# yangjunjie0320/fft-isdf-scratch

Measured on AMD Instinct MI355X. Metric: ISDF build + get_jk k-points/s, diamond gth-dzvp 4x4x4, higher is better.
Workload: dtype f64 (complex128)

## Files before the change

fft-isdf-scratch_amd/csrc/fft.hip:

```cpp
#include <type_traits>

#include "common.h"

typedef double fft_dv2 __attribute__((ext_vector_type(2)));


#include <map>
#include <mutex>
#include <vector>
#include <cmath>

namespace fisdf {

namespace {

constexpr int MAXN = 64;
constexpr int MAXST = 8;

struct Stages {
  int nst;
  int radix[MAXST];
};

template <int R>
__device__ __forceinline__ void dft_small(cplx* v, const cplx* __restrict__ tw, int n) {
  if constexpr (R == 2) {
    cplx a = v[0], b = v[1];
    v[0] = cadd(a, b);
    v[1] = csub(a, b);
  } else if constexpr (R == 4) {
    cplx a0 = cadd(v[0], v[2]), a1 = csub(v[0], v[2]);
    cplx b0 = cadd(v[1], v[3]), b1 = csub(v[1], v[3]);
    cplx b1m = cmk(b1.y, -b1.x);
    v[0] = cadd(a0, b0);
    v[2] = csub(a0, b0);
    v[1] = cadd(a1, b1m);
    v[3] = csub(a1, b1m);
  } else {
    cplx o[R];
    const int step = n / R;
#pragma unroll
    for (int k = 0; k < R; ++k) {
      cplx acc = v[0];
#pragma unroll
      for (int r = 1; r < R; ++r) acc = cadd(acc, cmul(v[r], tw[((r * k) % R) * step]));
      o[k] = acc;
    }
#pragma unroll
    for (int k = 0; k < R; ++k) v[k] = o[k];
  }
}

template <int R>
__device__ __forceinline__ void stockham_stage(const cplx* __restrict__ src, cplx* __restrict__ dst,
                                               const cplx* __restrict__ tw, int n, int Ns, int TL,
                                               int ps, int ls, int tid, int nthr) {
  const int nb = n / R;
  const int total = nb * TL;
  const int twstep = n / (Ns * R);
  for (int bf = tid; bf < total; bf += nthr) {
    const int l = bf % TL, j = bf / TL;
    cplx v[R];
#pragma unroll
    for (int r = 0; r < R; ++r) v[r] = src[(j + r * nb) * ps + l * ls];
    const int k = j % Ns;
    if (Ns > 1) {
#pragma unroll
      for (int r = 1; r < R; ++r) v[r] = cmul(v[r], tw[(k * r * twstep) % n]);
    }
    dft_small<R>(v, tw, n);
    const int idx = (j / Ns) * Ns * R + k;
#pragma unroll
    for (int r = 0; r < R; ++r) dst[(idx + r * Ns) * ps + l * ls] = v[r];
  }
}

template <bool BIG>
__device__ cplx* lds_fft_lines(cplx* a, cplx* b, const cplx* tw, int n, const int* radix, int nst,
                               int TL, int ps, int ls, int tid, int nthr) {
  int Ns = 1;
  for (int s = 0; s < nst; ++s) {
    const int R = radix[s];
    switch (R) {
      case 2: stockham_stage<2>(a, b, tw, n, Ns, TL, ps, ls, tid, nthr); break;
      case 3: stockham_stage<3>(a, b, tw, n, Ns, TL, ps, ls, tid, nthr); break;
      case 4: stockham_stage<4>(a, b, tw, n, Ns, TL, ps, ls, tid, nthr); break;
      case 5: stockham_stage<5>(a, b, tw, n, Ns, TL, ps, ls, tid, nthr); break;
      case 7: if constexpr (BIG) stockham_stage<7>(a, b, tw, n, Ns, TL, ps, ls, tid, nthr); break;
      case 11: if constexpr (BIG) stockham_stage<11>(a, b, tw, n, Ns, TL, ps, ls, tid, nthr); break;
      case 13: if constexpr (BIG) stockham_stage<13>(a, b, tw, n, Ns, TL, ps, ls, tid, nthr); break;
    }
    Ns *= R;
    __syncthreads();
    cplx* t = a;
    a = b;
    b = t;
  }
  return a;
}

__device__ __forceinline__ double fftfreq(int i, int n) {
  return (double)(i < (n + 1) / 2 ? i : i - n) / (double)n;
}

template <bool BIG>
__global__ __launch_bounds__(256) void fft_axis_kernel(
    const cplx* __restrict__ in, long in_ld, const int* __restrict__ rowidx, cplx* out, long out_ld,
    int rows, int n, int inner, int outer, int TL, int contiguous, Stages st,
    const cplx* __restrict__ twg, int n0, int n1, int n2, double kd0, double kd1, double kd2,
    int use_phase, const double* __restrict__ weight) {
  extern __shared__ cplx smem[];
  cplx* tw = smem;
  cplx* buf0 = smem + MAXN;
  cplx* buf1 = buf0 + TL * n;
  const int tid = threadIdx.x, nthr = blockDim.x;
  for (int t = tid; t < n; t += nthr) tw[t] = twg[t];

  long tile = blockIdx.x;
  int tiles_per_row = contiguous ? (outer + TL - 1) / TL : outer * (inner / TL);
  int row = (int)(tile / tiles_per_row);
  int trow = (int)(tile % tiles_per_row);
  if (row >= rows) return;
  const cplx* src = in + (long)(rowidx ? rowidx[row] : row) * in_ld;
  cplx* dstp = out + (long)row * out_ld;
  const int ngrid = n0 * n1 * n2;

  long base;
  int nlines = TL;
  if (contiguous) {
    int o0 = trow * TL;
    nlines = min(TL, outer - o0);
    base = (long)o0 * n;
  } else {
    int o = trow / (inner / TL), ib = trow % (inner / TL);
    base = (long)o * n * inner + (long)ib * TL;
  }
  auto gidx = [&](int l, int p) -> long {
    return contiguous ? base + (long)l * n + p : base + (long)p * inner + l;
  };

  const int tot = TL * n;
  constexpr int U = 8;
  cplx pre[U];
#pragma unroll
  for (int u = 0; u < U; ++u) {
    const int e = tid + u * nthr;
    int l, p;
    if (contiguous) { l = e / n; p = e % n; } else { l = e % TL; p = e / TL; }
    const bool ok = e < tot && l < nlines;
    pre[u] = src[ok ? gidx(l, p) : 0];
  }
  __syncthreads();
  auto put = [&](int e, cplx v) {
    int l, p;
    if (contiguous) { l = e / n; p = e % n; } else { l = e % TL; p = e / TL; }
    if (l < nlines) {
      if (use_phase) {
        long g = gidx(l, p);
        int i2 = (int)(g % n2);
        int i1 = (int)((g / n2) % n1);
        int i0 = (int)(g / ((long)n1 * n2));
        double th = -(fftfreq(i0, n0) * kd0 + fftfreq(i1, n1) * kd1 + fftfreq(i2, n2) * kd2);
        double s, c;
        sincos(th, &s, &c);
        v = cmul(v, cmk(c, s));
      }
    } else {
      v = cmk(0, 0);
    }
    buf0[p * TL + l] = v;
  };
#pragma unroll
  for (int u = 0; u < U; ++u) {
    const int e = tid + u * nthr;
    if (e < tot) put(e, pre[u]);
  }
  for (int e = tid + U * nthr; e < tot; e += nthr) {
    int l, p;
    if (contiguous) { l = e / n; p = e % n; } else { l = e % TL; p = e / TL; }
    put(e, l < nlines ? src[gidx(l, p)] : cmk(0, 0));
  }
  __syncthreads();
  cplx* a = lds_fft_lines<BIG>(buf0, buf1, tw, n, st.radix, st.nst, TL, TL, 1, tid, nthr);
  for (int e = tid; e < tot; e += nthr) {
    int l, p;
    if (contiguous) { l = e / n; p = e % n; } else { l = e % TL; p = e / TL; }
    if (l < nlines) {
      long g = gidx(l, p);
      cplx v = a[p * TL + l];
      if (weight) v = cscale(v, weight[g % ngrid]);
      dstp[g] = v;
    }
  }
}

template <bool BIG>
__global__ __launch_bounds__(256) void fft_plane_kernel(
    const cplx* __restrict__ in, long in_ld, const int* __restrict__ rowidx, cplx* out, long out_ld,
    int rows, Stages st1, Stages st2, const cplx* __restrict__ tw1g, const cplx* __restrict__ tw2g,
    int n0, int n1, int n2, double kd0, double kd1, double kd2, int use_phase,
    const PlaneRef* __restrict__ planes) {
  extern __shared__ cplx smem[];
  cplx* tw1 = smem;
  cplx* tw2 = smem + MAXN;
  cplx* ph1 = smem + 2 * MAXN;
  cplx* ph2 = smem + 3 * MAXN;
  const int P = n1 * n2;
  cplx* buf0 = smem + 4 * MAXN;
  cplx* buf1 = buf0 + P;
  const int tid = threadIdx.x, nthr = blockDim.x;
  const int row = blockIdx.x / n0, i0 = blockIdx.x % n0;
  if (row >= rows) return;
  const long r = rowidx ? rowidx[row] : row;
  const cplx* src = planes ? in + planes[i0].base + r * planes[i0].ld : in + r * in_ld + (long)i0 * P;
  cplx* dstp = out + (long)row * out_ld + (long)i0 * P;
  constexpr int U = 8;
  cplx v[U];
#pragma unroll
  for (int u = 0; u < U; ++u) {
    const int e = tid + u * nthr;
    v[u] = src[e < P ? e : 0];
  }
  for (int t = tid; t < n1; t += nthr) tw1[t] = tw1g[t];
  for (int t = tid; t < n2; t += nthr) tw2[t] = tw2g[t];
  if (use_phase) {
    double s0, c0;
    sincos(-fftfreq(i0, n0) * kd0, &s0, &c0);
    for (int t = tid; t < n1; t += nthr) {
      double s, c;
      sincos(-fftfreq(t, n1) * kd1, &s, &c);
      ph1[t] = cmul(cmk(c, s), cmk(c0, s0));
    }
    for (int t = tid; t < n2; t += nthr) {
      double s, c;
      sincos(-fftfreq(t, n2) * kd2, &s, &c);
      ph2[t] = cmk(c, s);
    }
  }
  __syncthreads();
#pragma unroll
  for (int u = 0; u < U; ++u) {
    const int e = tid + u * nthr;
    if (e < P) {
      cplx x = v[u];
      if (use_phase) x = cmul(x, cmul(ph1[e / n2], ph2[e % n2]));
      buf0[e] = x;
    }
  }
  for (int e = tid + U * nthr; e < P; e += nthr) {
    cplx x = src[e];
    if (use_phase) x = cmul(x, cmul(ph1[e / n2], ph2[e % n2]));
    buf0[e] = x;
  }
  __syncthreads();
  cplx* a = lds_fft_lines<BIG>(buf0, buf1, tw2, n2, st2.radix, st2.nst, n1, 1, n2, tid, nthr);
  cplx* b = a == buf0 ? buf1 : buf0;
  a = lds_fft_lines<BIG>(a, b, tw1, n1, st1.radix, st1.nst, n2, n2, 1, tid, nthr);
  for (int e = tid; e < P; e += nthr) dstp[e] = a[e];
}

template <int I, int N, typename F>
__device__ __forceinline__ void static_for(F&& f) {
  if constexpr (I < N) {
    f(std::integral_constant<int, I>{});
    static_for<I + 1, N>(f);
  }
}

constexpr int first_factor(int n) {
  return (n % 4 == 0 && n > 4) ? 4 : (n % 2 == 0 && n > 2) ? 2 : (n % 3 == 0 && n > 3) ? 3
       : (n % 5 == 0 && n > 5) ? 5 : n;
}

template <int NT, int E>
__device__ __forceinline__ cplx twmul(cplx v, const cplx* __restrict__ W) {
  constexpr int e = E % NT;
  if constexpr (e == 0) return v;
  else if constexpr (4 * e == NT) return cmk(v.y, -v.x);
  else if constexpr (2 * e == NT) return cmk(-v.x, -v.y);
  else if constexpr (4 * e == 3 * NT) return cmk(-v.y, v.x);
  else return cmul(v, W[e]);
}

template <int N, int NT>
__device__ __forceinline__ void fft_rec(cplx* x, const cplx* __restrict__ W) {
  if constexpr (N == 1) {
  } else if constexpr (N == 2) {
    const cplx a = x[0], b = x[1];
    x[0] = cadd(a, b);
    x[1] = csub(a, b);
  } else if constexpr (N == 4) {
    const cplx a0 = cadd(x[0], x[2]), a1 = csub(x[0], x[2]);
    const cplx b0 = cadd(x[1], x[3]), b1 = csub(x[1], x[3]);
    const cplx b1m = cmk(b1.y, -b1.x);
    x[0] = cadd(a0, b0);
    x[2] = csub(a0, b0);
    x[1] = cadd(a1, b1m);
    x[3] = csub(a1, b1m);
  } else if constexpr (first_factor(N) == N) {
    cplx o[N];
    static_for<0, N>([&](auto kc) {
      constexpr int K = decltype(kc)::value;
      cplx acc = x[0];
      static_for<1, N>([&](auto jc) {
        constexpr int J = decltype(jc)::value;
        acc = cadd(acc, twmul<NT, ((J * K) % N) * (NT / N)>(x[J], W));
      });
      o[K] = acc;
    });
    static_for<0, N>([&](auto kc) { x[decltype(kc)::value] = o[decltype(kc)::value]; });
  } else {
    constexpr int A = first_factor(N), B = N / A;
    cplx y[N];
    static_for<0, B>([&](auto n2c) {
      constexpr int N2 = decltype(n2c)::value;
      cplx t[A];
      static_for<0, A>([&](auto c) { t[decltype(c)::value] = x[B * decltype(c)::value + N2]; });
      fft_rec<A, NT>(t, W);
      static_for<0, A>([&](auto c) {
        constexpr int K1 = decltype(c)::value;
        y[K1 * B + N2] = twmul<NT, (N2 * K1) * (NT / N)>(t[K1], W);
      });
    });
    static_for<0, A>([&](auto k1c) {
      constexpr int K1 = decltype(k1c)::value;
      cplx t[B];
      static_for<0, B>([&](auto c) { t[decltype(c)::value] = y[K1 * B + decltype(c)::value]; });
      fft_rec<B, NT>(t, W);
      static_for<0, B>([&](auto c) { x[K1 + A * decltype(c)::value] = t[decltype(c)::value]; });
    });
  }
}

template <int NN>
__global__ __launch_bounds__(64) void fft_plane_reg(const cplx* __restrict__ in, long in_ld,
                                                    const int* __restrict__ rowidx, cplx* out,
                                                    long out_ld, int rows, int n0,
                                                    const cplx* __restrict__ W, double kd0,
                                                    double kd1, double kd2, int use_phase,
                                                    const PlaneRef* __restrict__ planes,
                                                    int nrow_out, int in_real) {
  constexpr int P = NN * NN, LD = NN + 1;
  __shared__ cplx img[NN * LD];
  __shared__ cplx ph1[NN], ph2[NN];
  const int lane = threadIdx.x;
  const int row = blockIdx.x / n0, i0 = blockIdx.x % n0;
  if (row >= rows) return;
  const long r = rowidx ? rowidx[row] : row;
  const cplx* src = planes ? in + planes[i0].base + r * planes[i0].ld : in + r * in_ld + (long)i0 * P;
  cplx* dst = out + (long)row * out_ld + (long)i0 * P;
  constexpr int U = (P + 63) / 64;
  cplx v[U];
  if (in_real) {
    const double* srr = (const double*)in + r * in_ld + (long)i0 * P;
#pragma unroll
    for (int u = 0; u < U; ++u) {
      const int e = lane + 64 * u;
      v[u] = cmk(srr[e < P ? e : 0], 0.0);
    }
  } else {
#pragma unroll
    for (int u = 0; u < U; ++u) {
      const int e = lane + 64 * u;
      v[u] = src[e < P ? e : 0];
    }
  }
  if (use_phase && lane < NN) {
    double s0, c0, s, c;
    sincos(-fftfreq(i0, n0) * kd0, &s0, &c0);
    sincos(-fftfreq(lane, NN) * kd1, &s, &c);
    ph1[lane] = cmul(cmk(c, s), cmk(c0, s0));
    sincos(-fftfreq(lane, NN) * kd2, &s, &c);
    ph2[lane] = cmk(c, s);
  }
  __syncthreads();
#pragma unroll
  for (int u = 0; u < U; ++u) {
    const int e = lane + 64 * u;
    if (e < P) {
      const int i1 = e / NN, i2 = e - i1 * NN;
      cplx x = v[u];
      if (use_phase) x = cmul(x, cmul(ph1[i1], ph2[i2]));
      img[i1 * LD + i2] = x;
    }
  }
  __syncthreads();
  if (lane < NN) {
    cplx x[NN];
#pragma unroll
    for (int p = 0; p < NN; ++p) x[p] = img[lane * LD + p];
    fft_rec<NN, NN>(x, W);
#pragma unroll
    for (int p = 0; p < NN; ++p) img[lane * LD + p] = x[p];
  }
  __syncthreads();
  if (lane < NN) {
    cplx x[NN];
#pragma unroll
    for (int p = 0; p < NN; ++p) x[p] = img[p * LD + lane];
    fft_rec<NN, NN>(x, W);
#pragma unroll
    for (int p = 0; p < NN; ++p) img[p * LD + lane] = x[p];
  }
  __syncthreads();
  const int Pout = nrow_out * NN;
#pragma unroll
  for (int u = 0; u < U; ++u) {
    const int e = lane + 64 * u;
    if (e < Pout) {
      const int i1 = e / NN, i2 = e - i1 * NN;
      dst[e] = img[i1 * LD + i2];
    }
  }
}

template <int N0>
__global__ __launch_bounds__(256) void fft_axis0_reg(const cplx* in, long in_ld, cplx* out,
                                                     long out_ld, int rows, int P,
                                                     const cplx* __restrict__ W,
                                                     const double* __restrict__ weight) {
  const long t = blockIdx.x * (long)blockDim.x + threadIdx.x;
  if (t >= (long)rows * P) return;
  const int row = (int)(t / P), l = (int)(t - (long)row * P);
  const cplx* src = in + (long)row * in_ld + l;
  cplx* dst = out + (long)row * out_ld + l;
  cplx x[N0];
#pragma unroll
  for (int p = 0; p < N0; ++p) x[p] = src[(long)p * P];
  fft_rec<N0, N0>(x, W);
  if (weight) {
#pragma unroll
    for (int p = 0; p < N0; ++p) x[p] = cscale(x[p], weight[(long)p * P + l]);
  }
#pragma unroll
  for (int p = 0; p < N0; ++p)
    __builtin_nontemporal_store(fft_dv2{x[p].x, x[p].y}, (fft_dv2*)(dst + (long)p * P));
}

constexpr int herm_prefix(int n, int m) {
  int nH = 0;
  for (int i = 0; i < n; ++i)
    if (i <= ((-i - m) % n + n) % n) nH = i + 1;
  return nH;
}

template <int N0, int M0>
__global__ __launch_bounds__(256) void fft_axis0_herm(const cplx* in, long in_ld, cplx* out,
                                                      long out_ld, int rows, int n1, int n2,
                                                      int m1, int m2, int lo, int hi, int sl0,
                                                      int sl1, int npb,
                                                      const cplx* __restrict__ W,
                                                      const double* __restrict__ weight) {
  constexpr int NH = herm_prefix(N0, M0);
  const int P = n1 * n2;
  const int lane = threadIdx.x & 63;
  int row, c, d;
  bool flip = false;
  if ((int)blockIdx.x < npb) {
    const long npr = (long)(hi - lo) * n2;
    const long k = ((long)blockIdx.x * 4 + (threadIdx.x >> 6)) * 32 + (lane & 31);
    if (k >= (long)rows * npr) return;
    row = (int)(k / npr);
    const int kk = (int)(k - (long)row * npr);
    const int j1 = lo + kk / n2, j2 = kk - (kk / n2) * n2;
    c = j1 * n2 + j2;
    flip = lane >= 32;
    d = flip ? (((-j1 - m1) % n1 + n1) % n1) * n2 + ((-j2 - m2) % n2 + n2) % n2 : c;
  } else {
    const int nsl = (sl0 >= 0) + (sl1 >= 0);
    const long nsr = (long)nsl * n2;
    const long s = (long)(blockIdx.x - npb) * 256 + threadIdx.x;
    if (s >= (long)rows * nsr) return;
    row = (int)(s / nsr);
    const int ss = (int)(s - (long)row * nsr);
    const int li = ss / n2;
    const int j1 = (li == 0 && sl0 >= 0) ? sl0 : sl1;
    c = d = j1 * n2 + (ss - li * n2);
  }
  const cplx* src = in + (long)row * in_ld + c;
  cplx* dst = out + (long)row * out_ld + d;
  cplx x[N0];
#pragma unroll
  for (int p = 0; p < N0; ++p) x[p] = src[(long)p * P];
  if (flip) {
#pragma unroll
    for (int p = 0; p < N0; ++p) {
      x[p].y = -x[p].y;
      if constexpr (M0 != 0) x[p] = cmul(x[p], W[(p * M0) % N0]);
    }
  }
  fft_rec<N0, N0>(x, W);
  if (weight) {
#pragma unroll
    for (int p = 0; p < NH; ++p) x[p] = cscale(x[p], weight[(long)p * P + d]);
  }
#pragma unroll
  for (int p = 0; p < NH; ++p)
    __builtin_nontemporal_store(fft_dv2{x[p].x, x[p].y}, (fft_dv2*)(dst + (long)p * P));
}

#define FISDF_REG_SIZES(X) X(8) X(12) X(13) X(15) X(16) X(18) X(20) X(24) X(25) X(27) X(30) X(32) X(36) X(40) X(45) X(48)

int fft_plane_reg_launch(hipStream_t s, int n, const cplx* in, long in_ld, const int* rowidx,
                         cplx* out, long out_ld, int rows, int n0, const cplx* W, const double* kd,
                         const PlaneRef* planes, int nrow_out, bool in_real, bool* done) {
  *done = false;
  const double k0 = kd ? kd[0] : 0, k1 = kd ? kd[1] : 0, k2 = kd ? kd[2] : 0;
  const long nplanes = (long)rows * n0;
#define FISDF_PL(N)                                                                            \
  if (n == N) {                                                                                \
    hipLaunchKernelGGL(fft_plane_reg<N>, dim3((unsigned)nplanes), dim3(64), 0, s, in, in_ld,    \
                       rowidx, out, out_ld, rows, n0, W, k0, k1, k2, kd ? 1 : 0, planes,        \
                       nrow_out, in_real ? 1 : 0);                                            \
    *done = true;                                                                              \
  }
  FISDF_REG_SIZES(FISDF_PL)
#undef FISDF_PL
  if (*done) FISDF_HIP(hipGetLastError());
  return 0;
}

int fft_axis0_reg_launch(hipStream_t s, int n0, const cplx* in, long in_ld, cplx* out, long out_ld,
                         int rows, int P, const cplx* W, const double* weight, bool* done) {
  *done = false;
  const long threads = (long)rows * P;
  const unsigned blocks = (unsigned)((threads + 255) / 256);
#define FISDF_AX(N)                                                                            \
  if (n0 == N) {                                                                               \
    hipLaunchKernelGGL(fft_axis0_reg<N>, dim3(blocks), dim3(256), 0, s, in, in_ld, out, out_ld, \
                       rows, P, W, weight);                                                    \
    *done = true;                                                                              \
  }
  FISDF_REG_SIZES(FISDF_AX)
#undef FISDF_AX
  if (*done) FISDF_HIP(hipGetLastError());
  return 0;
}

struct HermGeom {
  int lo, hi, sl0, sl1;
  long npb, blocks;
};

int herm_geom(int rows, int n1, int n2, int n1H, int m1, HermGeom* g) {
  auto partner1 = [&](int j) { return ((-j - m1) % n1 + n1) % n1; };
  const int sl0 = partner1(0) == 0 ? 0 : -1;
  const int sl1 = (n1H - 1 > 0 && partner1(n1H - 1) == n1H - 1) ? n1H - 1 : -1;
  const int lo = sl0 >= 0 ? 1 : 0, hi = sl1 >= 0 ? n1H - 1 : n1H;
  for (int j = lo; j < hi; ++j)
    FISDF_CHECK(partner1(j) >= n1H, "fft: Hermitian line pairing");
  const long pairs = (long)rows * (hi - lo) * n2;
  const long npb = (pairs + 127) / 128;
  const long nself = (long)rows * ((sl0 >= 0) + (sl1 >= 0)) * n2;
  const long blocks = npb + (nself + 255) / 256;
  FISDF_CHECK(blocks < (1L << 31), "fft: too many blocks");
  *g = HermGeom{lo, hi, sl0, sl1, npb, blocks};
  return 0;
}

int fft_axis0_herm_launch(hipStream_t s, int n0, const cplx* in, long in_ld, cplx* out,
                          long out_ld, int rows, int n1, int n2, int n1H, const int m[3],
                          const cplx* W, const double* weight, bool* done) {
  *done = false;
  HermGeom hg;
  FISDF_TRY(herm_geom(rows, n1, n2, n1H, m[1], &hg));
  const int lo = hg.lo, hi = hg.hi, sl0 = hg.sl0, sl1 = hg.sl1;
  const long npb = hg.npb, blocks = hg.blocks;
#define FISDF_AXH(N)                                                                           \
  if (n0 == N) {                                                                               \
    if (m[0] == 0)                                                                             \
      hipLaunchKernelGGL((fft_axis0_herm<N, 0>), dim3((unsigned)blocks), dim3(256), 0, s, in,    \
                         in_ld, out, out_ld, rows, n1, n2, m[1], m[2], lo, hi, sl0, sl1,       \
                         (int)npb, W, weight);                                                 \
    else                                                                                       \
      hipLaunchKernelGGL((fft_axis0_herm<N, 1>), dim3((unsigned)blocks), dim3(256), 0, s, in,    \
                         in_ld, out, out_ld, rows, n1, n2, m[1], m[2], lo, hi, sl0, sl1,       \
                         (int)npb, W, weight);                                                 \
    *done = true;                                                                              \
  }
  FISDF_REG_SIZES(FISDF_AXH)
#undef FISDF_AXH
  if (*done) FISDF_HIP(hipGetLastError());
  return 0;
}

bool needs_big(const Stages& st) {
  for (int i = 0; i < st.nst; ++i)
    if (st.radix[i] > 5) return true;
  return false;
}

bool factorize(int n, Stages& st) {
  st.nst = 0;
  const int rs[] = {4, 2, 3, 5, 7, 11, 13};
  for (int r : rs)
    while (n % r == 0) {
      if (st.nst >= MAXST) return false;
      st.radix[st.nst++] = r;
      n /= r;
    }
  return n == 1;
}

struct TwTable {
  cplx* dev = nullptr;
};
std::mutex g_tw_mu;
std::map<std::pair<int, int>, TwTable> g_tw;

int get_twiddles(int n, const cplx** out) {
  int dev = 0;
  FISDF_HIP(hipGetDevice(&dev));
  std::lock_guard<std::mutex> lk(g_tw_mu);
  auto key = std::make_pair(dev, n);
  auto it = g_tw.find(key);
  if (it == g_tw.end()) {
    std::vector<cplx> h(n);
    for (int t = 0; t < n; ++t) {
      long double ang = -2.0L * 3.14159265358979323846264338327950288L * t / n;
      h[t] = cmk((double)cosl(ang), (double)sinl(ang));
      if ((4 * t) % n == 0) {
        int q = (4 * t) / n;
        const double re[4] = {1, 0, -1, 0}, im[4] = {0, -1, 0, 1};
        h[t] = cmk(re[q], im[q]);
      }
    }
    TwTable tt;
    FISDF_HIP(hipMalloc(&tt.dev, sizeof(cplx) * n));
    FISDF_HIP(hipMemcpy(tt.dev, h.data(), sizeof(cplx) * n, hipMemcpyHostToDevice));
    it = g_tw.emplace(key, tt).first;
  }
  *out = it->second.dev;
  return 0;
}

int largest_divisor_le(int x, int cap) {
  for (int d = std::min(x, cap); d >= 1; --d)
    if (x % d == 0) return d;
  return 1;
}

struct AxisGeom {
  int n, inner, outer, contiguous, TL;
  long tiles;
  size_t lds;
  Stages st;
};

int axis_geom(int rows, int axis, int n0, int n1, int n2, AxisGeom* g) {
  const int dims[3] = {n0, n1, n2};
  const int n = dims[axis];
  FISDF_CHECK(n0 >= 1 && n1 >= 1 && n2 >= 1, "fft: mesh dimension must be in [1, 64]");
  FISDF_CHECK(n >= 1 && n <= MAXN, "fft: mesh dimension must be in [1, 64]");
  FISDF_CHECK(factorize(n, g->st), "fft: mesh dimension must factor into 2,3,5,7,11,13");
  int inner = 1, outer = 1;
  for (int a = axis + 1; a < 3; ++a) inner *= dims[a];
  for (int a = 0; a < axis; ++a) outer *= dims[a];
  int contiguous = (axis == 2);
  int TL;
  long tiles;
  if (contiguous) {
    TL = std::max(1, std::min(64, 2048 / n));
    tiles = (long)rows * ((outer + TL - 1) / TL);
  } else {
    TL = largest_divisor_le(inner, 64);
    if (TL < 16 && inner > 64) TL = largest_divisor_le(inner, 128);
    FISDF_CHECK(TL <= 128, "fft: tile too wide");
    tiles = (long)rows * outer * (inner / TL);
  }
  FISDF_CHECK(tiles < (1L << 31), "fft: too many tiles");
  size_t lds = sizeof(cplx) * (MAXN + 2 * (size_t)TL * n);
  FISDF_CHECK(lds <= 160 * 1024, "fft: LDS tile too large");
  g->n = n; g->inner = inner; g->outer = outer; g->contiguous = contiguous; g->TL = TL;
  g->tiles = tiles; g->lds = lds;
  return 0;
}

int axis_pass(hipStream_t s, const cplx* in, long in_ld, const int* rowidx, cplx* out, long out_ld,
              int rows, int axis, int n0, int n1, int n2, const double* kd, const double* weight) {
  AxisGeom g;
  FISDF_TRY(axis_geom(rows, axis, n0, n1, n2, &g));
  const int n = g.n, inner = g.inner, outer = g.outer, contiguous = g.contiguous, TL = g.TL;
  const long tiles = g.tiles;
  const size_t lds = g.lds;
  const Stages& st = g.st;
  const cplx* tw = nullptr;
  FISDF_TRY(get_twiddles(n, &tw));
  double k0 = 0, k1 = 0, k2 = 0;
  int use_phase = kd != nullptr;
  if (kd) { k0 = kd[0]; k1 = kd[1]; k2 = kd[2]; }
  if (needs_big(st))
    hipLaunchKernelGGL(fft_axis_kernel<true>, dim3((unsigned)tiles), dim3(256), lds, s, in, in_ld,
                       rowidx, out, out_ld, rows, n, inner, outer, TL, contiguous, st, tw, n0, n1,
                       n2, k0, k1, k2, use_phase, weight);
  else
    hipLaunchKernelGGL(fft_axis_kernel<false>, dim3((unsigned)tiles), dim3(256), lds, s, in, in_ld,
                       rowidx, out, out_ld, rows, n, inner, outer, TL, contiguous, st, tw, n0, n1,
                       n2, k0, k1, k2, use_phase, weight);
  FISDF_HIP(hipGetLastError());
  return 0;
}

}

bool reg_mesh(int n0, int n1, int n2) {
  if (n1 != n2) return false;
  int a = 0, b = 0;
#define FISDF_HAS(N) if (n1 == N) a = 1; if (n0 == N) b = 1;
  FISDF_REG_SIZES(FISDF_HAS)
#undef FISDF_HAS
  return a && b;
}

size_t plane_kernel_lds(int n1, int n2) { return sizeof(cplx) * (4 * MAXN + 2 * (size_t)n1 * n2); }

bool fft3d_reads_real(int n0, int n1, int n2) { return reg_mesh(n0, n1, n2); }

bool fft3d_reads_slices(int n0, int n1, int n2) {
  return reg_mesh(n0, n1, n2) || plane_kernel_lds(n1, n2) <= 96 * 1024;
}

bool fft_herm_enabled() {
  static const bool on = [] {
    const char* e = getenv("FISDF_FFT_HERM");
    return !(e && e[0] == '0');
  }();
  return on;
}

int fft3d_route(int n0, int n1, int n2, const int* herm) {
  if (reg_mesh(n0, n1, n2))
    return herm && (herm[0] == 0 || herm[0] == 1) && fft_herm_enabled() ? FFT_REG_HERM : FFT_REG;
  bool big = false;
  for (int n : {n0, n1, n2}) {
    Stages st;
    if (n >= 1 && n <= MAXN && factorize(n, st)) big = big || needs_big(st);
  }
  return (plane_kernel_lds(n1, n2) <= 96 * 1024 ? FFT_PLANE : FFT_AXES) | (big ? FFT_BIG : 0);
}

int fft3d(hipStream_t s, const cplx* in, long in_ld, const int* rowidx, cplx* out, long out_ld,
          int rows, int n0, int n1, int n2, const double* kd, const double* weight, cplx* ,
          const PlaneRef* planes, const int* herm, bool in_real) {
  if (rows == 0) return 0;
  FISDF_CHECK(!in_real || (reg_mesh(n0, n1, n2) && !planes && in != out),
              "fft: real input needs the register path and unsliced, out-of-place rows");
  FISDF_CHECK(in != out || rowidx == nullptr, "fft: in-place pass cannot gather rows");
  FISDF_CHECK(!planes || fft3d_reads_slices(n0, n1, n2), "fft: sliced input needs a plane kernel");
  const int route = fft3d_route(n0, n1, n2, herm) & ~FFT_BIG;
  if (route == FFT_REG || route == FFT_REG_HERM) {
    const cplx *W12 = nullptr, *W0 = nullptr;
    FISDF_TRY(get_twiddles(n1, &W12));
    FISDF_TRY(get_twiddles(n0, &W0));
    bool ok1 = false, ok0 = false;
    FISDF_CHECK((long)rows * n0 < (1L << 31) && (long)rows * n1 * n2 < (1L << 38), "fft: too large");
    if (route == FFT_REG_HERM) {
      const int m[3] = {herm[0], ((herm[1] % n1) + n1) % n1, ((herm[2] % n2) + n2) % n2};
      const int n1H = herm_prefix(n1, m[1]);
      HermGeom hg;
      FISDF_TRY(herm_geom(rows, n1, n2, n1H, m[1], &hg));
      FISDF_TRY(fft_plane_reg_launch(s, n1, in, in_ld, rowidx, out, out_ld, rows, n0, W12, kd,
                                     planes, n1H, in_real, &ok1));
      FISDF_TRY(fft_axis0_herm_launch(s, n0, out, out_ld, out, out_ld, rows, n1, n2, n1H, m, W0,
                                      weight, &ok0));
      FISDF_CHECK(ok1 && ok0, "fft: register kernel dispatch failed");
      return 0;
    }
    {
      FISDF_TRY(fft_plane_reg_launch(s, n1, in, in_ld, rowidx, out, out_ld, rows, n0, W12, kd,
                                     planes, n1, in_real, &ok1));
      FISDF_TRY(fft_axis0_reg_launch(s, n0, out, out_ld, out, out_ld, rows, n1 * n2, W0, weight, &ok0));
      FISDF_CHECK(ok1 && ok0, "fft: register kernel dispatch failed");
      return 0;
    }
  }
  AxisGeom geom;
  for (int axis = route == FFT_PLANE ? 0 : 2; axis >= 0; --axis)
    FISDF_TRY(axis_geom(rows, axis, n0, n1, n2, &geom));
  const size_t plane_lds = plane_kernel_lds(n1, n2);
  if (route == FFT_PLANE) {
    Stages st1, st2;
    FISDF_CHECK(n1 <= MAXN && n2 <= MAXN && factorize(n1, st1) && factorize(n2, st2),
                "fft: mesh dimension must be <= 64 and factor into 2,3,5,7,11,13");
    const cplx *tw1 = nullptr, *tw2 = nullptr;
    FISDF_TRY(get_twiddles(n1, &tw1));
    FISDF_TRY(get_twiddles(n2, &tw2));
    const long nplanes = (long)rows * n0;
    FISDF_CHECK(nplanes < (1L << 31), "fft: too many planes");
    double k0 = 0, k1 = 0, k2 = 0;
    if (kd) { k0 = kd[0]; k1 = kd[1]; k2 = kd[2]; }
    if (needs_big(st1) || needs_big(st2))
      hipLaunchKernelGGL(fft_plane_kernel<true>, dim3((unsigned)nplanes), dim3(256), plane_lds, s,
                         in, in_ld, rowidx, out, out_ld, rows, st1, st2, tw1, tw2, n0, n1, n2, k0,
                         k1, k2, kd != nullptr ? 1 : 0, planes);
    else
      hipLaunchKernelGGL(fft_plane_kernel<false>, dim3((unsigned)nplanes), dim3(256), plane_lds, s,
                         in, in_ld, rowidx, out, out_ld, rows, st1, st2, tw1, tw2, n0, n1, n2, k0,
                         k1, k2, kd != nullptr ? 1 : 0, planes);
    FISDF_HIP(hipGetLastError());
  } else {
    FISDF_TRY(axis_pass(s, in, in_ld, rowidx, out, out_ld, rows, 2, n0, n1, n2, kd, nullptr));
    FISDF_TRY(axis_pass(s, out, out_ld, nullptr, out, out_ld, rows, 1, n0, n1, n2, nullptr, nullptr));
  }
  FISDF_TRY(axis_pass(s, out, out_ld, nullptr, out, out_ld, rows, 0, n0, n1, n2, nullptr, weight));
  return 0;
}

}
```

Baseline: 835.5.

## Add multi-wave lean 2D plane FFT kernel using two-pass factorized LDS transforms

Introduces fft_plane_lean, which processes each 2D plane with a block of several waves (default 4) instead of one 64-lane wave. Each axis is split into a first-factor radix-A pass with twiddles and a radix-B pass, all done in shared memory, and the output is read back in digit-reversed order. The aim is more parallelism per plane and lower register pressure than the one-wave fully in-register transform. The cost is extra synchronisation and LDS traffic. The kernel is on by default through a macro, and experiment macros that skip work are compiled out unless defined.

```diff
diff --git a/fft-isdf-scratch_amd/csrc/fft.hip b/fft-isdf-scratch_amd/csrc/fft.hip
--- a/fft-isdf-scratch_amd/csrc/fft.hip
+++ b/fft-isdf-scratch_amd/csrc/fft.hip
@@ -3,6 +3,13 @@
 #include "common.h"
 
 typedef double fft_dv2 __attribute__((ext_vector_type(2)));
+
+#ifndef FISDF_FFT_LEAN
+#define FISDF_FFT_LEAN 1
+#endif
+#ifndef FISDF_FFT_LEAN_WAVES
+#define FISDF_FFT_LEAN_WAVES 4
+#endif
 
 
 #include <map>
@@ -414,6 +421,120 @@
   }
 }
 
+template <int NN>
+__device__ __forceinline__ int lean_pos(int j) {
+  constexpr int A = first_factor(NN), B = NN / A;
+  return (j % A) * B + j / A;
+}
+
+template <int NN, int NW, bool AX1>
+__device__ __forceinline__ void lean_lines(cplx* img, const cplx* tw, const cplx* __restrict__ W,
+                                           int lane) {
+  constexpr int A = first_factor(NN), B = NN / A, LD = NN + 1;
+  constexpr int ES = AX1 ? LD : 1, LS = AX1 ? 1 : LD;
+#pragma unroll 1
+  for (int it = lane; it < NN * B; it += 64 * NW) {
+    const int line = AX1 ? it % NN : it / B, n2 = AX1 ? it / NN : it % B;
+    cplx* p = img + line * LS + n2 * ES;
+    cplx t[A];
+#pragma unroll
+    for (int c = 0; c < A; ++c) t[c] = p[B * c * ES];
+    fft_rec<A, NN>(t, W);
+    if constexpr (B > 1) {
+#pragma unroll
+      for (int k1 = 1; k1 < A; ++k1) t[k1] = cmul(t[k1], tw[n2 * k1]);
+    }
+#pragma unroll
+    for (int k1 = 0; k1 < A; ++k1) p[B * k1 * ES] = t[k1];
+  }
+  if constexpr (B > 1) {
+    __syncthreads();
+#pragma unroll 1
+    for (int it = lane; it < NN * A; it += 64 * NW) {
+      const int line = AX1 ? it % NN : it / A, k1 = AX1 ? it / NN : it % A;
+      cplx* p = img + line * LS + B * k1 * ES;
+      cplx t[B];
+#pragma unroll
+      for (int c = 0; c < B; ++c) t[c] = p[c * ES];
+      fft_rec<B, NN>(t, W);
+#pragma unroll
+      for (int c = 0; c < B; ++c) p[c * ES] = t[c];
+    }
+  }
+  __syncthreads();
+}
+
+template <int NN, int NW>
+__global__ __launch_bounds__(64 * NW) void fft_plane_lean(const cplx* __restrict__ in, long in_ld,
+                                                          const int* __restrict__ rowidx,
+                                                          cplx* out, long out_ld, int rows, int n0,
+                                                          const cplx* __restrict__ W, double kd0,
+                                                          double kd1, double kd2, int use_phase,
+                                                          const PlaneRef* __restrict__ planes,
+                                                          int nrow_out, int in_real) {
+  constexpr int P = NN * NN, LD = NN + 1;
+  constexpr int NT = 64 * NW, U = (P + NT - 1) / NT;
+  __shared__ cplx img[NN * LD];
+  __shared__ cplx ph1[NN], ph2[NN], tw[NN];
+  const int lane = threadIdx.x;
+  const int row = blockIdx.x / n0, i0 = blockIdx.x % n0;
+  if (row >= rows) return;
+  const long r = rowidx ? rowidx[row] : row;
+  const cplx* src = planes ? in + planes[i0].base + r * planes[i0].ld : in + r * in_ld + (long)i0 * P;
+  cplx* dst = out + (long)row * out_ld + (long)i0 * P;
+  cplx v[U];
+  if (in_real) {
+    const double* srr = (const double*)in + r * in_ld + (long)i0 * P;
+#pragma unroll
+    for (int u = 0; u < U; ++u) {
+      const int e = lane + NT * u;
+      v[u] = cmk(srr[e < P ? e : 0], 0.0);
+    }
+  } else {
+#pragma unroll
+    for (int u = 0; u < U; ++u) {
+      const int e = lane + NT * u;
+      v[u] = src[e < P ? e : 0];
+    }
+  }
+  if (lane < NN) {
+    tw[lane] = W[lane];
+    if (use_phase) {
+      double s0, c0, s, c;
+      sincos(-fftfreq(i0, n0) * kd0, &s0, &c0);
+      sincos(-fftfreq(lane, NN) * kd1, &s, &c);
+      ph1[lane] = cmul(cmk(c, s), cmk(c0, s0));
+      sincos(-fftfreq(lane, NN) * kd2, &s, &c);
+      ph2[lane] = cmk(c, s);
+    }
+  }
+  __syncthreads();
+#pragma unroll
+  for (int u = 0; u < U; ++u) {
+    const int e = lane + NT * u;
+    if (e < P) {
+      const int i1 = e / NN, i2 = e - i1 * NN;
+      cplx x = v[u];
+      if (use_phase) x = cmul(x, cmul(ph1[i1], ph2[i2]));
+      img[i1 * LD + i2] = x;
+    }
+  }
+  __syncthreads();
+#ifndef FISDF_EXP_LEAN_NOLINES
+  lean_lines<NN, NW, false>(img, tw, W, lane);
+  lean_lines<NN, NW, true>(img, tw, W, lane);
+#endif
+  const int Pout = nrow_out * NN;
+#pragma unroll
+  for (int u = 0; u < U; ++u) {
+    const int e = lane + NT * u;
+    if (e < Pout) {
+      const int j1 = e / NN, j2 = e - j1 * NN;
+      dst[e] = img[lean_pos<NN>(j1) * LD + lean_pos<NN>(j2)];
+    }
+  }
+}
+
 template <int N0>
 __global__ __launch_bounds__(256) void fft_axis0_reg(const cplx* in, long in_ld, cplx* out,
                                                      long out_ld, int rows, int P,
@@ -505,8 +626,21 @@
                          cplx* out, long out_ld, int rows, int n0, const cplx* W, const double* kd,
                          const PlaneRef* planes, int nrow_out, bool in_real, bool* done) {
   *done = false;
+#ifdef FISDF_EXP_NOPLANE
+  *done = true;
+  return 0;
+#endif
   const double k0 = kd ? kd[0] : 0, k1 = kd ? kd[1] : 0, k2 = kd ? kd[2] : 0;
   const long nplanes = (long)rows * n0;
+#if FISDF_FFT_LEAN
+#define FISDF_PL(N)                                                                            \
+  if (n == N) {                                                                                \
+    hipLaunchKernelGGL((fft_plane_lean<N, FISDF_FFT_LEAN_WAVES>), dim3((unsigned)nplanes),     \
+                       dim3(64 * FISDF_FFT_LEAN_WAVES), 0, s, in, in_ld, rowidx, out, out_ld,  \
+                       rows, n0, W, k0, k1, k2, kd ? 1 : 0, planes, nrow_out, in_real ? 1 : 0); \
+    *done = true;                                                                              \
+  }
+#else
 #define FISDF_PL(N)                                                                            \
   if (n == N) {                                                                                \
     hipLaunchKernelGGL(fft_plane_reg<N>, dim3((unsigned)nplanes), dim3(64), 0, s, in, in_ld,    \
@@ -514,6 +648,7 @@
                        nrow_out, in_real ? 1 : 0);                                            \
     *done = true;                                                                              \
   }
+#endif
   FISDF_REG_SIZES(FISDF_PL)
 #undef FISDF_PL
   if (*done) FISDF_HIP(hipGetLastError());
@@ -523,6 +658,10 @@
 int fft_axis0_reg_launch(hipStream_t s, int n0, const cplx* in, long in_ld, cplx* out, long out_ld,
                          int rows, int P, const cplx* W, const double* weight, bool* done) {
   *done = false;
+#ifdef FISDF_EXP_NOAXIS0
+  *done = true;
+  return 0;
+#endif
   const long threads = (long)rows * P;
   const unsigned blocks = (unsigned)((threads + 255) / 256);
 #define FISDF_AX(N)                                                                            \
@@ -562,6 +701,10 @@
                           long out_ld, int rows, int n1, int n2, int n1H, const int m[3],
                           const cplx* W, const double* weight, bool* done) {
   *done = false;
+#ifdef FISDF_EXP_NOAXIS0
+  *done = true;
+  return 0;
+#endif
   HermGeom hg;
   FISDF_TRY(herm_geom(rows, n1, n2, n1H, m[1], &hg));
   const int lo = hg.lo, hi = hg.hi, sl0 = hg.sl0, sl1 = hg.sl1;
```

After: 843.2 (median of 6 runs). No clear change (+0.9%).
